# ajingu/RealSenseCalibration

Measured on NVIDIA B200. Metric: LM iterations/sec, higher is better.
Workload: dtype f64

## Files before the change

realsensecalibration_b200/csrc/ba_cuda.cu:

```cuda
#include <dlfcn.h>

#include <algorithm>
#include <atomic>
#include <chrono>
#include <cmath>
#include <string>

#include "ba_dense.cuh"
#include "ba_dense_blocked.cuh"
#include "ba_kernels.cuh"
#include "ba_structure.cuh"
#include "ba_rcs.cuh"
#include "ba_fused_a.cuh"
#include "ba_strip_a.cuh"
#include "ba_exchange.cuh"
#include "ba_rig.cuh"
#include "ba_cov.cuh"

using namespace ba;

namespace {
typedef struct ncclComm* ncclComm_t;
struct NcclUniqueId { char internal[128]; };
struct Nccl {
// ... 495 lines not shown
  }
  BA_LAUNCH(p, KT_CANDIDATE, (k_candidate<6>), gcf, 256, 0, S.nf, p->f_act_ptr.p, p->xf.p, p->sf.p, p->yf.p, p->xf_c.p, p->bp0.p, p->bp1.p);
  {
    FoldJob J = {{p->bp0.p, p->bp1.p, nullptr, nullptr}, {S_XF2, S_DF2, 0, 0}, {0, 0, 0, 0}};
    BA_LAUNCH(p, KT_FOLD, k_fold_multi, 2, 1024, 0, J, gcf, p->scal.p);
  }
  BA_CUDA_TRY(cudaGetLastError());
  fam_end(p, F_UPDATE);
  fam_begin(p, F_COST);
  BA_TRY(run_cost_candidate(p));
  fam_end(p, F_COST);
  return allreduce_step_scalars(p);
}

FaParams fa_params(ba_cuda_problem* p, const ba_cuda_options& opt) {
  const Structure& S = p->S;
  FusedA& F = p->FA;
  const size_t nt = (size_t)F.n_tiles;
  FaParams P;
  P.tiles = F.tiles.p; P.e_ptr = S.e_ptr.p; P.ob_f = S.ob_f0.p; P.uv = p->uv.p;
  P.ob_meta = p->use_strip ? p->SA.ob_meta.p : F.ob_meta.p;
  P.tile_cams = p->use_strip ? p->SA.strip_cams.p : F.cams.group_target.p; P.cap = F.cap;
  P.pts_cap = F.pts_cap; P.tcam = F.tcam; P.tcs = F.tcs; P.pent_cap = F.pent_cap;
  P.pitem_begin = F.pairs.item_begin.p; P.pitem_end = F.pairs.item_end.p; P.pent = F.pairs.ent.p;
  P.citem_begin = F.cams.item_begin.p; P.citem_end = F.cams.item_end.p; P.cent = F.cams.ent.p;
  P.xe = p->xe.p; P.se = p->se.p; P.tab_f = p->tab_f.p; P.radius = p->scal.p + S_RADIUS;
  P.min_diag = opt.min_lm_diagonal; P.max_diag = opt.max_lm_diagonal;
  P.partP = F.partP.p; P.partC = F.partC.p; P.Lz = F.Lz.p; P.se_out = p->se.p;
  P.cost_partial = p->fa_part.p; P.g2_partial = p->fa_part.p + nt; P.gmax_partial = p->fa_part.p + 2 * nt;
  P.yf = p->yf.p; P.tabc_f = p->tabc_f.p; P.xe_c = p->xe_c.p;
  P.mcc_partial = p->fa_part.p + 3 * nt; P.x2_partial = p->fa_part.p + 4 * nt; P.d2_partial = p->fa_part.p + 5 * nt;
  P.cand_partial = p->fa_part.p + 6 * nt;
  P.RES = p->RES.p; P.JE = p->JE.p; P.JF = p->JF0.p;
  P.status = p->status.p;
  P.loss = p->loss;
  return P;
}

int fa_set_smem_attr(ba_cuda_problem* p) {
  if (!p->smem_attr_set) {
    const int kMax = (int)FA_SMEM_MAX;
    BA_CUDA_TRY(cudaFuncSetAttribute(k_fa_pass1<FA_FULL>, cudaFuncAttributeMaxDynamicSharedMemorySize, kMax));
    BA_CUDA_TRY(cudaFuncSetAttribute(k_fa_pass1<FA_NORMS>, cudaFuncAttributeMaxDynamicSharedMemorySize, kMax));
    BA_CUDA_TRY(cudaFuncSetAttribute(k_fa_pass1<FA_GRAD>, cudaFuncAttributeMaxDynamicSharedMemorySize, kMax));
    BA_CUDA_TRY(cudaFuncSetAttribute(k_fa_pass1<FA_FIRST>, cudaFuncAttributeMaxDynamicSharedMemorySize, kMax));
    BA_CUDA_TRY(cudaFuncSetAttribute(k_fa_pass2, cudaFuncAttributeMaxDynamicSharedMemorySize, kMax));
    BA_CUDA_TRY(cudaFuncSetAttribute(k_fa_jac, cudaFuncAttributeMaxDynamicSharedMemorySize, kMax));
    BA_CUDA_TRY(cudaFuncSetAttribute(k_sa_pass1<SA_FULL>, cudaFuncAttributeMaxDynamicSharedMemorySize, kMax));
    BA_CUDA_TRY(cudaFuncSetAttribute(k_sa_pass1<SA_GRAD>, cudaFuncAttributeMaxDynamicSharedMemorySize, kMax));
    BA_CUDA_TRY(cudaFuncSetAttribute(k_sa_pass1<SA_FIRST>, cudaFuncAttributeMaxDynamicSharedMemorySize, kMax));
    p->smem_attr_set = true;
  }
  return BA_OK;
}

// ... 201 lines not shown
      LaunchScope scope(p, KT_RCS);
      BA_TRY(launch_pcg(p->pcg, p->R, p->Sb.p, p->rhs.p, p->yf.p, p->status.p, opt, p->st));
    }
    BA_CUDA_TRY(cudaMemcpyAsync(&p->h_pcg_iters, p->pcg.iters.p, sizeof(int), cudaMemcpyDeviceToHost, p->st));
  } else {
    if (p->use_strip)
      BA_LAUNCH(p, KT_ASSEMBLE, k_sa_diag_rhs_dense, grid_for(S.nf * 6, 128), 128, 0, S.nf, F.camacc.p, radius, opt.min_lm_diagonal,
                opt.max_lm_diagonal, n, p->Sd.p, p->rhs.p);
    else
      BA_LAUNCH(p, KT_ASSEMBLE, k_diag_rhs_dense, grid_for(S.nf * 6, 128), 128, 0, S.nf, F.camacc.p, FA_NVC, F.camacc.p + 27, FA_NVC, radius,
                opt.min_lm_diagonal, opt.max_lm_diagonal, n, p->Sd.p, p->rhs.p);
    LaunchScope scope(p, KT_RCS);
    BA_TRY(dense_solve(p, n));
  }
  fam_end(p, F_SOLVE);
  fam_begin(p, F_UPDATE);
  const int gcf = (int)grid_for(S.nf * 6, 256);
  BA_LAUNCH(p, KT_CANDIDATE, (k_candidate<6>), gcf, 256, 0, S.nf, p->f_act_ptr.p, p->xf.p, p->sf.p, p->yf.p, p->xf_c.p, p->bp0.p, p->bp1.p);
  {
    FoldJob J = {{p->bp0.p, p->bp1.p, nullptr, nullptr}, {S_XF2, S_DF2, 0, 0}, {0, 0, 0, 0}};
    BA_LAUNCH(p, KT_FOLD, k_fold_multi, 2, 1024, 0, J, gcf, p->scal.p);
  }
  BA_TRY(build_tables(p, true));
  const FaParams P = fa_params(p, opt);
  BA_LAUNCH(p, KT_FA_P2, k_fa_pass2, F.n_tiles, F.threads2, F.smem2(), P);
  {
    FoldJob J = {{P.mcc_partial, P.x2_partial, P.d2_partial, P.cand_partial}, {S_MCC, S_XE2, S_DE2, S_CAND}, {0, 0, 0, 0}};
    BA_LAUNCH(p, KT_FOLD, k_fold_multi, 4, 1024, 0, J, F.n_tiles, p->scal.p);
  }
  BA_CUDA_TRY(cudaGetLastError());
  fam_end(p, F_UPDATE);
  return allreduce_step_scalars(p);
}

bool lm_fused(const ba_cuda_problem* p) { return p->model == 0 && p->use_fused && !p->lm.opt.force_generic_path; }

int sx_prepare(ba_cuda_problem* p) {
  const Structure& S = p->S;
  SparseExchange& X = p->SX;
  X.on = false; X.world = p->world; X.nvc = p->use_strip ? SA_NVC : FA_NVC;
  if (!nccl().AllGather || !env_int("BA_SX", 0, 1, 1)) return BA_OK;
  cudaStream_t st = p->st;
  const int64_t nf = S.nf, nd = p->R.nd;
  DVec<int32_t> cflag, cpos, dflag, dpos;
  BA_TRY(cflag.alloc(nf + 1)); BA_TRY(cpos.alloc(nf + 1)); BA_TRY(dflag.alloc((size_t)S.ndest + 1)); BA_TRY(dpos.alloc((size_t)S.ndest + 1));
  BA_CUDA_TRY(cudaMemsetAsync(cflag.p, 0, sizeof(int32_t) * (nf + 1), st));
  BA_CUDA_TRY(cudaMemsetAsync(dflag.p, 0, sizeof(int32_t) * ((size_t)S.ndest + 1), st));
  k_sx_flags<<<grid_for(nf, 256), 256, 0, st>>>(S.fobs_ptr.p, nf, cflag.p);
// ... 1424 lines not shown
```

realsensecalibration_b200/csrc/ba_fused_a.cuh:

```cuda
#pragma once
#include <cuda_pipeline.h>

#include <chrono>
#include <cstdio>

#include "ba_kernels.cuh"
#include "ba_structure.cuh"

namespace ba {

constexpr int FA_TOBS_DEFAULT = 256;
constexpr int FA_KMAX = 64;
constexpr int FA_TPTS = 4096;
constexpr int FA_TCAM = 48;
constexpr int FA_CH_PAIR = 16;
constexpr int FA_CH_RED = 64;
constexpr int FA_NVC = 33;
constexpr int FA_MAX_THREADS = 512;
constexpr int FA_THREADS_DEFAULT = 128;
constexpr int FA_REC = 22;
constexpr int FA_REC2 = 10;
constexpr int FA_PENT_MAX = 6144;
constexpr size_t FA_SMEM_MAX = 231000;
constexpr int FA_LS = 10;
// ... 42 lines not shown
  DVec<int64_t> tile_item_ptr;
  DVec<int32_t> item_target;
  DVec<int32_t> red_items;
  DVec<int64_t> tgt_ptr;
  Chunks red_ch;
  DVec<int64_t> group_ptr;
  DVec<int32_t> group_target;
  DVec<int64_t> tile_group_ptr;
};

struct FusedA {
  bool ready = false;
  int n_tiles = 0, tobs = FA_TOBS_DEFAULT, kmax = 0, cap = 0, threads = FA_THREADS_DEFAULT, threads2 = FA_THREADS_DEFAULT, ch_cam = 16, ch_pair = FA_CH_PAIR;
  DVec<int64_t> tile_pt_ptr;
  DVec<int64_t> tile_pent_ptr;
  DVec<int64_t> tile_cent_ptr;
  ItemSet pairs, cams;
  DVec<uint32_t> ob_meta;
  DVec<FaTile> tiles;
  DVec<double> partP, partC, red1P, red1C, camacc, Lz;
  int pts_cap = FA_TPTS;
  int tcam = FA_TCAM;
  int tcs = FA_TCAM + 1;
  int pent_cap = 0;
  size_t smem1() const {
    return ((size_t)cap * FA_REC + (size_t)pts_cap * FA_LS + (size_t)tcs * TAB) * 8 + ((size_t)pent_cap + cap) * 4 + (size_t)cap * 2;
  }
  size_t smem2() const { return ((size_t)cap * FA_REC2 + (size_t)pts_cap * FA_PS2 + (size_t)tcs * (TAB + 16)) * 8; }
  size_t smemj(int threads) const { return ((size_t)threads * FA_RECJ + (size_t)pts_cap * FA_PS2 + (size_t)tcs * TAB) * 8 + (size_t)cap * 20; }
};

__global__ void k_fa_tile_flags(const int64_t* __restrict__ e_ptr, int64_t ne, int tobs, int32_t* __restrict__ flag, int* __restrict__ kmax) {
  const int64_t pt = blockIdx.x * (int64_t)blockDim.x + threadIdx.x;
  if (pt >= ne) return;
  atomicMax(kmax, (int)min(e_ptr[pt + 1] - e_ptr[pt], (int64_t)INT32_MAX));
  int f = 0;
  if (pt > 0) f = (e_ptr[pt] / tobs != e_ptr[pt - 1] / tobs) || (pt / FA_TPTS != (pt - 1) / FA_TPTS);
  flag[pt] = f;
}

__global__ void k_fa_pair_fill(const int64_t* __restrict__ e_ptr, const int32_t* __restrict__ ob_f, int64_t ne, int64_t nf,
                               const int64_t* __restrict__ off, const int32_t* __restrict__ tile_of_pt, const int64_t* __restrict__ tile_pt_ptr,
                               const uint64_t* __restrict__ dest_keys, int ndest, const uint64_t* __restrict__ dh_keys,
                               const int32_t* __restrict__ dh_val, uint64_t dh_mask, int dh_shift, uint64_t* __restrict__ keys,
                               int32_t* __restrict__ vals) {
  const int64_t e = blockIdx.x * (int64_t)blockDim.x + threadIdx.x;
  if (e >= ne) return;
  int64_t o = off[e];
  const int tile = tile_of_pt[e];
  const int64_t ob0 = e_ptr[tile_pt_ptr[tile]];
  for (int64_t i = e_ptr[e]; i < e_ptr[e + 1]; ++i)
// ... 256 lines not shown
inline int build_fused_a_tobs(FusedA& F, const Structure& S, cudaStream_t st, int tobs);

inline int build_fused_a(FusedA& F, const Structure& S, cudaStream_t st) {
  F.ready = false;
  if (S.ne == 0 || S.nb == 0 || S.nslots != 1) return BA_ERR_UNSUPPORTED;
  const int64_t np = S.npairs - S.nf;
  if (np >= (int64_t)INT32_MAX) return BA_ERR_UNSUPPORTED;
  const bool dense_pairs = (double)np >= 4.0 * (double)S.nb;
  int tobs = env_int("BA_FA_TOBS", 64, 1024, dense_pairs ? 1024 : 480);
  for (;; tobs /= 2) {
    F.threads = env_int("BA_FA_THREADS", 32, FA_MAX_THREADS, tobs >= 768 ? 512 : 256) / 32 * 32;
    F.threads2 = env_int("BA_FA_THREADS2", 32, FA_MAX_THREADS, tobs >= 768 ? 256 : 128) / 32 * 32;
    F.ch_cam = env_int("BA_FA_CH_CAM", 1, 63, 16);
    F.ch_pair = env_int("BA_FA_CH_PAIR", 1, 63, dense_pairs ? FA_CH_PAIR : 12);
    const int rc = build_fused_a_tobs(F, S, st, tobs);
    if (rc != BA_ERR_UNSUPPORTED || tobs <= 128 || F.kmax > FA_KMAX) return rc;
  }
}

inline int build_fused_a_tobs(FusedA& F, const Structure& S, cudaStream_t st, int tobs) {
  F.ready = false;
  const int64_t ne = S.ne, nb = S.nb, nf = S.nf;
  F.tobs = tobs;
  FaLap L(st);
  DVec<int32_t> flag, tile_of_pt;
  DVec<int> kmax;
  BA_TRY(flag.alloc(ne)); BA_TRY(tile_of_pt.alloc(ne)); BA_TRY(kmax.alloc_zero(1, st));
  k_fa_tile_flags<<<grid_for(ne, 256), 256, 0, st>>>(S.e_ptr.p, ne, F.tobs, flag.p, kmax.p);
  BA_TRY(cub_call([&](void* t, size_t& b) { return cub::DeviceScan::InclusiveSum(t, b, flag.p, tile_of_pt.p, (int)ne, st); }));
  int last_tile = 0;
  BA_CUDA_TRY(cudaMemcpyAsync(&F.kmax, kmax.p, sizeof(int), cudaMemcpyDeviceToHost, st));
  BA_CUDA_TRY(cudaMemcpyAsync(&last_tile, tile_of_pt.p + (ne - 1), sizeof(int32_t), cudaMemcpyDeviceToHost, st));
  BA_CUDA_TRY(cudaStreamSynchronize(st));
  if (F.kmax > FA_KMAX) return BA_ERR_UNSUPPORTED;
  F.cap = F.tobs + F.kmax;
  F.n_tiles = last_tile + 1;
  BA_TRY(F.tile_pt_ptr.alloc((size_t)F.n_tiles + 1));
  k_seg_ptr<int32_t><<<grid_for(ne > F.n_tiles + 1 ? ne : F.n_tiles + 1, 256), 256, 0, st>>>(tile_of_pt.p, ne, F.n_tiles, F.tile_pt_ptr.p);
  L.lap("tiles");
  int max_tile_cams = 0;
  {
    DVec<uint64_t> keys;
    DVec<int32_t> vals, group_tile;
    DVec<int> mx;
    BA_TRY(keys.alloc(nb)); BA_TRY(vals.alloc(nb)); BA_TRY(mx.alloc_zero(1, st));
    k_fa_cam_fill<<<grid_for(nb, 256), 256, 0, st>>>(S.ob_e.p, S.ob_f0.p, nb, nf, S.e_ptr.p, tile_of_pt.p, F.tile_pt_ptr.p, keys.p, vals.p);
// ... 62 lines not shown
    F.tcs = F.tcam | 1;
    F.pent_cap = std::min(h[2], FA_PENT_MAX);
    F.pent_cap += F.pent_cap & 1;
    if (F.smem1() > FA_SMEM_MAX) {
      const size_t excess = (F.smem1() - FA_SMEM_MAX + 7) / 8 * 2;
      F.pent_cap = (size_t)F.pent_cap > excess ? F.pent_cap - (int)excess : 0;
    }
    if (F.smem1() > FA_SMEM_MAX || F.smem2() > FA_SMEM_MAX || F.smemj(FA_JAC_THREADS) > FA_SMEM_MAX) return BA_ERR_UNSUPPORTED;
  }
  L.lap("pair items, geometry");
  BA_TRY(F.tiles.alloc((size_t)F.n_tiles));
  k_fa_tile_desc<<<grid_for(F.n_tiles, 256), 256, 0, st>>>(F.n_tiles, F.tile_pt_ptr.p, S.e_ptr.p, F.cams.tile_group_ptr.p, F.tile_pent_ptr.p,
                                                          F.tile_cent_ptr.p, F.pairs.tile_item_ptr.p, F.cams.tile_item_ptr.p, F.tiles.p);
  BA_TRY(F.partP.alloc((size_t)F.pairs.n_items * 36)); BA_TRY(F.partC.alloc((size_t)F.cams.n_items * FA_NVC));
  BA_TRY(F.red1P.alloc((size_t)F.pairs.red_ch.n * 36)); BA_TRY(F.red1C.alloc((size_t)F.cams.red_ch.n * FA_NVC));
  BA_TRY(F.camacc.alloc((size_t)nf * FA_NVC + 2 + 64));
  BA_TRY(F.Lz.alloc((size_t)ne * 9));
  BA_CUDA_TRY(cudaStreamSynchronize(st));
  BA_CUDA_TRY(cudaGetLastError());
  F.ready = true;
  return BA_OK;
}

__device__ __forceinline__ void fa_linearize(const double* __restrict__ T, const double* X, const double* s, double2 ob, double* r,
                                             double* je, double* jf) {
  double q[3];
  mat3_vec(T, X, q);
  const double p0 = q[0] + T[18], p1 = q[1] + T[19], p2 = q[2] + T[20];
  r[0] = T[21] * p0 / p2 + T[23] - ob.x;
  r[1] = T[22] * p1 / p2 + T[24] - ob.y;
  const double iz = 1.0 / p2;
  const double a = T[21] * iz, bb = -T[21] * p0 * iz * iz, cc = T[22] * iz, dd = -T[22] * p1 * iz * iz;
  double D[9];
  rot_deriv(T + 9, T[25] != 0.0 ? X : q, D);
#pragma unroll
  for (int k = 0; k < 3; ++k) {
    jf[k] = (a * D[k] + bb * D[6 + k]) * T[26 + k];
    jf[6 + k] = (cc * D[3 + k] + dd * D[6 + k]) * T[26 + k];
  }
  jf[3] = a * T[29]; jf[4] = 0.0;        jf[5] = bb * T[31];
  jf[9] = 0.0;       jf[10] = cc * T[30]; jf[11] = dd * T[31];
  je[0] = (a * T[0] + bb * T[6]) * s[0]; je[1] = (a * T[1] + bb * T[7]) * s[1]; je[2] = (a * T[2] + bb * T[8]) * s[2];
  je[3] = (cc * T[3] + dd * T[6]) * s[0]; je[4] = (cc * T[4] + dd * T[7]) * s[1]; je[5] = (cc * T[5] + dd * T[8]) * s[2];
}

__device__ __forceinline__ bool fa_chol3(const double* M , double* Lp) {
  const double d0 = M[0];
  if (!(d0 > 0.0) || !isfinite(d0)) return false;
  const double i0 = rsqrt(d0);
  const double l10 = M[1] * i0, l20 = M[2] * i0;
  const double d1 = M[3] - l10 * l10;
  if (!(d1 > 0.0) || !isfinite(d1)) return false;
  const double i1 = rsqrt(d1);
  const double l21 = (M[4] - l20 * l10) * i1;
  const double d2 = M[5] - l20 * l20 - l21 * l21;
  if (!(d2 > 0.0) || !isfinite(d2)) return false;
  Lp[0] = l10; Lp[1] = l20; Lp[2] = l21; Lp[3] = i0; Lp[4] = i1; Lp[5] = rsqrt(d2);
  return true;
}
__device__ __forceinline__ void fa_fwd3(const double* Lp, double* x) {
  x[0] *= Lp[3];
  x[1] = (x[1] - Lp[0] * x[0]) * Lp[4];
  x[2] = (x[2] - Lp[1] * x[0] - Lp[2] * x[1]) * Lp[5];
}
__device__ __forceinline__ void fa_bwd3(const double* Lp, double* x) {
  x[2] *= Lp[5];
  x[1] = (x[1] - Lp[2] * x[2]) * Lp[4];
  x[0] = (x[0] - Lp[0] * x[1] - Lp[1] * x[2]) * Lp[3];
}

struct FaParams {
  const FaTile* tiles;
  const int64_t* e_ptr; const int32_t* ob_f; const uint32_t* ob_meta; const double2* uv;
  const int32_t* tile_cams;
  const int64_t* pitem_begin; const int64_t* pitem_end; const int32_t* pent;
  const int64_t* citem_begin; const int64_t* citem_end; const int32_t* cent;
  int cap, pts_cap, tcam, tcs, pent_cap;
  const double* xe; const double* se; const double* tab_f; const double* radius;
  double min_diag, max_diag;
  double* partP; double* partC; double* Lz; double* se_out;
  double* cost_partial; double* gmax_partial; double* g2_partial;
  const double* yf; const double* tabc_f; double* xe_c;
  double* mcc_partial; double* x2_partial; double* d2_partial; double* cand_partial;
  double* RES; double* JE; double* JF;
  int* status;
  LossSpec loss;
};

__device__ __forceinline__ double fa_apply_loss(const LossSpec L, double* r, double* je, double* jf) {
  const double s = r[0] * r[0] + r[1] * r[1];
  if (L.type == 0) return s;
  double rho, w;
  loss_apply(L, s, &rho, &w);
  r[0] *= w; r[1] *= w;
#pragma unroll
  for (int k = 0; k < 6; ++k) je[k] *= w;
#pragma unroll
  for (int k = 0; k < 12; ++k) jf[k] *= w;
  return rho;
}

__device__ __forceinline__ FaTile fa_load_tile(const FaTile* __restrict__ p) {
  FaTile T;
  const int4* s = reinterpret_cast<const int4*>(p);
  int4* d = reinterpret_cast<int4*>(&T);
#pragma unroll
// ... 266 lines not shown
      const double2 rv = R2[9], wv = R2[10];
      int c = 0;
#pragma unroll
      for (int a = 0; a < 6; ++a)
#pragma unroll
        for (int b = a; b < 6; ++b) acc[c++] += jf[a] * jf[b] + jf[6 + a] * jf[6 + b];
#pragma unroll
      for (int a = 0; a < 6; ++a) { acc[21 + a] += jf[a] * rv.x + jf[6 + a] * rv.y; acc[27 + a] += jf[a] * wv.x + jf[6 + a] * wv.y; }
    }
    double* out = P.partC + (size_t)it * FA_NVC;
#pragma unroll
    for (int k = 0; k < FA_NVC; ++k) out[k] = acc[k];
  }
  if (!NORMS) {
    double v[3] = {sq, g2, gmx};
    const bool mx[3] = {false, false, true};
    fa_block_reduce(v, mx, 3, red);
    if (tid == 0) { P.cost_partial[tile] = v[0]; P.g2_partial[tile] = v[1]; P.gmax_partial[tile] = v[2]; }
  }
}

__device__ __constant__ int kFaCandFields[16] = {0, 1, 2, 3, 4, 5, 6, 7, 8, 18, 19, 20, 21, 22, 23, 24};

__global__ void __launch_bounds__(FA_MAX_THREADS, 1) k_fa_pass2(FaParams P) {
  extern __shared__ double smem[];
  double* rec = smem;
  double* Xs = rec + (size_t)P.cap * FA_REC2;
  double* tabs = Xs + (size_t)P.pts_cap * FA_PS2;
  double* tabc = tabs + (size_t)P.tcs * TAB;
  __shared__ double red[128];
  const int tile = blockIdx.x, tid = threadIdx.x, nthr = blockDim.x;
  const FaTile T = fa_load_tile(P.tiles + tile);
  const int64_t pt0 = T.pt0, ob0 = T.ob0;
  const int nobs = T.nobs, npts = T.npts;
  fa_stage_tables_async(P, T, P.tab_f, tabs, TAB, nullptr);
  for (int i = tid; i < 3 * npts; i += nthr) {
    const int lp = i / 3, k = i - 3 * lp;
    __pipeline_memcpy_async(Xs + lp * FA_PS2 + k, P.xe + 3 * pt0 + i, 8);
    __pipeline_memcpy_async(Xs + lp * FA_PS2 + 3 + k, P.se + 3 * pt0 + i, 8);
  }
  __pipeline_commit();
  fa_stage_tables_async(P, T, P.tabc_f, tabc, 16, kFaCandFields);
  __pipeline_commit();
  int pl0 = 0, pl1 = 0;
  if (tid < npts) {
    pl0 = (int)(P.e_ptr[pt0 + tid] - ob0);
    pl1 = (int)(P.e_ptr[pt0 + tid + 1] - ob0);
  }
  uint32_t m_n = 0;
  int32_t c_n = 0;
  double2 uv_n = make_double2(0.0, 0.0);
  if (tid < nobs) { m_n = P.ob_meta[ob0 + tid]; c_n = P.ob_f[ob0 + tid]; uv_n = P.uv[ob0 + tid]; }
  __pipeline_wait_prior(1);
  __syncthreads();
  for (int l = tid; l < nobs; l += nthr) {
    const int lp = (int)(m_n & 0xffffu), slot = (int)(m_n >> 16);
    const int32_t c = c_n;
    const double2 ob = uv_n;
    if (l + nthr < nobs) { const int64_t o = ob0 + l + nthr; m_n = P.ob_meta[o]; c_n = P.ob_f[o]; uv_n = P.uv[o]; }
    double y[6];
#pragma unroll
    for (int k = 0; k < 6; ++k) y[k] = __ldg(P.yf + 6 * (int64_t)c + k);
    double Tt[TAB];
    fa_get_table(P, tabs, P.tab_f, slot, c, Tt);
    const double* xs = Xs + lp * FA_PS2;
    const double X[3] = {xs[0], xs[1], xs[2]};
    const double s[3] = {xs[3], xs[4], xs[5]};
    double r[2], je[6], jf[12];
    fa_linearize(Tt, X, s, ob, r, je, jf);
    fa_apply_loss(P.loss, r, je, jf);
    double q0 = 0.0, q1 = 0.0;
#pragma unroll
    for (int k = 0; k < 6; ++k) { q0 += jf[k] * y[k]; q1 += jf[6 + k] * y[k]; }
    double2* R2 = reinterpret_cast<double2*>(rec + (size_t)l * FA_REC2);
#pragma unroll
    for (int k = 0; k < 3; ++k) R2[k] = make_double2(je[2 * k], je[2 * k + 1]);
    R2[3] = make_double2(r[0], r[1]);
    R2[4] = make_double2(q0, q1);
  }
  uint32_t m2 = 0;
  double2 uv2 = make_double2(0.0, 0.0);
  if (tid < nobs) { m2 = P.ob_meta[ob0 + tid]; uv2 = P.uv[ob0 + tid]; }
  __syncthreads();
  double mcc = 0.0, x2 = 0.0, d2 = 0.0;
  for (int lp = tid; lp < npts; lp += nthr) {
    const int64_t e = pt0 + lp;
    int l0 = pl0, l1 = pl1;
    if (lp != tid) { l0 = (int)(P.e_ptr[e] - ob0); l1 = (int)(P.e_ptr[e + 1] - ob0); }
    const double* in = P.Lz + 9 * e;
    double Lp[6], t[3];
#pragma unroll
    for (int k = 0; k < 6; ++k) Lp[k] = in[k];
#pragma unroll
    for (int k = 0; k < 3; ++k) t[k] = in[6 + k];
    for (int l = l0; l < l1; ++l) {
      const double* R = rec + (size_t)l * FA_REC2;
#pragma unroll
      for (int rr = 0; rr < 2; ++rr) {
        double u[3] = {R[3 * rr], R[3 * rr + 1], R[3 * rr + 2]};
        fa_fwd3(Lp, u);
        const double q = R[8 + rr];
        t[0] -= u[0] * q; t[1] -= u[1] * q; t[2] -= u[2] * q;
      }
    }
    fa_bwd3(Lp, t);
    for (int l = l0; l < l1; ++l) {
      const double* R = rec + (size_t)l * FA_REC2;
#pragma unroll
      for (int rr = 0; rr < 2; ++rr) {
        const double m = -(R[3 * rr] * t[0] + R[3 * rr + 1] * t[1] + R[3 * rr + 2] * t[2]) - R[8 + rr];
        mcc += m * (R[6 + rr] + m / 2.0);
      }
    }
    double* xs = Xs + lp * FA_PS2;
#pragma unroll
    for (int k = 0; k < 3; ++k) {
      const double xv = xs[k];
      const double c = xv + (-(t[k]) * xs[3 + k]);
      P.xe_c[3 * e + k] = c;
      xs[k] = c;
      if (l1 > l0) { x2 += xv * xv; const double d = xv - c; d2 += d * d; }
    }
  }
  __pipeline_wait_prior(0);
  __syncthreads();
  double sq = 0.0;
  for (int l = tid; l < nobs; l += nthr) {
    const int lp = (int)(m2 & 0xffffu), slot = (int)(m2 >> 16);
    const double2 ob = uv2;
    if (l + nthr < nobs) { const int64_t o = ob0 + l + nthr; m2 = P.ob_meta[o]; uv2 = P.uv[o]; }
    double C[16];
    if (slot < P.tcam) {
#pragma unroll
      for (int f = 0; f < 16; ++f) C[f] = fa_table_field(tabc, P.tcs, f, slot);
    } else {
      const double* Tc = P.tabc_f + TAB * (int64_t)P.ob_f[ob0 + l];
#pragma unroll
      for (int f = 0; f < 16; ++f) C[f] = __ldg(Tc + kFaCandFields[f]);
    }
    const double* xs = Xs + lp * FA_PS2;
    const double X[3] = {xs[0], xs[1], xs[2]};
    double q[3];
    mat3_vec(C, X, q);
    const double p0 = q[0] + C[9], p1 = q[1] + C[10], p2 = q[2] + C[11];
    const double r0 = C[12] * p0 / p2 + C[14] - ob.x;
    const double r1 = C[13] * p1 / p2 + C[15] - ob.y;
    double sc = r0 * r0 + r1 * r1;
    if (P.loss.type != 0) { double w; loss_apply(P.loss, sc, &sc, &w); }
    sq += sc;
  }
  double v[4] = {mcc, x2, d2, sq};
  const bool mx[4] = {false, false, false, false};
  fa_block_reduce(v, mx, 4, red);
  if (tid == 0) { P.mcc_partial[tile] = v[0]; P.x2_partial[tile] = v[1]; P.d2_partial[tile] = v[2]; P.cand_partial[tile] = v[3]; }
}

__global__ void __launch_bounds__(FA_JAC_THREADS, 4) k_fa_jac(FaParams P) {
  extern __shared__ double smem[];
  const int tile = blockIdx.x, tid = threadIdx.x, nthr = blockDim.x, lane = tid & 31, warp = tid >> 5;
  double* wje = smem + (size_t)warp * (32 * FA_RECJ);
  double* wjf = wje + 32 * 6;
  double2* uv_s = reinterpret_cast<double2*>(smem + (size_t)(nthr >> 5) * (32 * FA_RECJ));
  double* Xs = reinterpret_cast<double*>(uv_s + P.cap);
  double* tabs = Xs + (size_t)P.pts_cap * FA_PS2;
  uint32_t* meta_s = reinterpret_cast<uint32_t*>(tabs + (size_t)P.tcs * TAB);
  __shared__ double red[32];
  const FaTile T = fa_load_tile(P.tiles + tile);
  const int64_t pt0 = T.pt0, ob0 = T.ob0;
  const int nobs = T.nobs, npts = T.npts;
  fa_stage_tables_async(P, T, P.tab_f, tabs, TAB, nullptr);
  for (int i = tid; i < 3 * npts; i += nthr) {
    const int lp = i / 3, k = i - 3 * lp;
    __pipeline_memcpy_async(Xs + lp * FA_PS2 + k, P.xe + 3 * pt0 + i, 8);
    __pipeline_memcpy_async(Xs + lp * FA_PS2 + 3 + k, P.se + 3 * pt0 + i, 8);
  }
  for (int i = tid; i < nobs; i += nthr) {
    __pipeline_memcpy_async(uv_s + i, P.uv + ob0 + i, 16);
// ... 140 lines not shown
```

realsensecalibration_b200/csrc/ba_strip_a.cuh:

```cuda
#pragma once
#include "ba_fused_a.cuh"

namespace ba {

constexpr int SA_NT = 512;
constexpr int SA_NCS_MAX = 64;
constexpr int SA_NVC = 39;
constexpr int SA_REC = 22;
constexpr int SA_NF_CAP = 1024;
constexpr int SA_POS_MAX = 4096;
constexpr int SA_CM_MAX = 8;
constexpr int SA_TYPE_IDLE = 0, SA_TYPE_PAIR = 1, SA_TYPE_FLUSH = 2, SA_TYPE_CAM = 3;
constexpr int SA_FULL = 0, SA_GRAD = 2, SA_FIRST = 3;

__host__ __device__ inline int sa_xs_len(int pts_cap) { return (3 * pts_cap + 4 + 1) & ~1; }

struct __align__(16) SaTile {
  int64_t pt0, ob0, pos0, ent0, pidx0, fout0;
  int32_t npts, nobs, npos, nent;
};
static_assert(sizeof(SaTile) == 64, "SaTile is loaded as four 16-byte words");
struct __align__(16) SaStrip {
  int64_t cam0, pout0, cout0;
  int32_t tile0, ntiles, ncs, nflush;
// ... 770 lines not shown
  const int64_t n_pblocks = A.n_pout + A.n_fout;
  if (n_pblocks >= (int64_t)INT32_MAX / 64 || A.n_cout >= (int64_t)INT32_MAX / 64) return BA_ERR_UNSUPPORTED;
  {
    DVec<int32_t> ptarget, ctarget, iota;
    BA_TRY(ptarget.alloc((size_t)n_pblocks)); BA_TRY(ctarget.alloc((size_t)A.n_cout));
    k_sa_targets_persist<<<grid_for((int64_t)ns * SA_NT, 256), 256, 0, st>>>(ns, A.strips.p, A.slot_out.p, slot_dest.p, A.strip_cams.p, nf,
                                                                            S.dh_keys.p, S.dh_val.p, S.dh_mask, S.dh_shift, ptarget.p, ctarget.p);
    k_sa_targets_flush<<<grid_for(nt, 4), 128, 0, st>>>(nt, L, A.segw, nf_cap, A.tiles.p, A.strips.p, A.seg.p, fl_dest.p, A.strip_cams.p, nf,
                                                       S.dh_keys.p, S.dh_val.p, S.dh_mask, S.dh_shift, A.n_pout, ptarget.p);
    const int64_t nmax = std::max(n_pblocks, A.n_cout);
    BA_TRY(iota.alloc((size_t)nmax));
    k_iota<<<grid_for(nmax, 256), 256, 0, st>>>(iota.p, nmax, 0);
    BA_TRY(sort_to_csr(ptarget.p, iota.p, n_pblocks, S.ndest, A.tgt_ptr_p, A.red_items_p, st));
    BA_TRY(build_chunks(A.red_ch_p, A.tgt_ptr_p.p, S.ndest, FA_CH_RED, st));
    BA_TRY(sort_to_csr(ctarget.p, iota.p, A.n_cout, nf, A.tgt_ptr_c, A.red_items_c, st));
    BA_TRY(build_chunks(A.red_ch_c, A.tgt_ptr_c.p, (int)nf, FA_CH_RED, st));
    BA_CUDA_TRY(cudaStreamSynchronize(st));
  }
  Lp.lap("strip: reduction lists");
  BA_TRY(A.partP.alloc((size_t)n_pblocks * 36)); BA_TRY(A.partC.alloc((size_t)A.n_cout * SA_NVC));
  BA_TRY(A.red1P.alloc((size_t)A.red_ch_p.n * 36)); BA_TRY(A.red1C.alloc((size_t)A.red_ch_c.n * SA_NVC));
  F.n_tiles = nt; F.tobs = tobs; F.kmax = A.kmax; F.cap = std::max(A.nobs_cap, 1);
  F.threads = SA_NT; F.threads2 = env_int("BA_FA_THREADS2", 32, FA_MAX_THREADS, tobs >= 640 ? 256 : 128) / 32 * 32;
  F.pts_cap = A.pts_cap; F.tcam = std::min(A.ncs_cap, FA_TCAM); F.tcs = F.tcam | 1; F.pent_cap = 0;
  if (F.smem2() > FA_SMEM_MAX || F.smemj(FA_JAC_THREADS) > FA_SMEM_MAX) return BA_ERR_UNSUPPORTED;
  BA_TRY(F.tiles.alloc((size_t)nt));
  k_sa_fa_tiles<<<grid_for(nt, 256), 256, 0, st>>>(nt, L, A.tiles.p, A.strips.p, F.tiles.p);
  BA_TRY(F.camacc.alloc((size_t)nf * SA_NVC + 2 + 64));
  BA_TRY(F.Lz.alloc((size_t)ne * 9));
  BA_CUDA_TRY(cudaStreamSynchronize(st));
  BA_CUDA_TRY(cudaGetLastError());
  if (Lp.on)
    std::fprintf(stderr, "[ba_cuda timing]   strip geometry: tobs %d L %d tiles %d strips %d | positions %d points %d cameras %d entries staged %d of %d "
                         "owner slots %d | smem %zu B | blocks: %lld per strip + %lld flushed, %lld camera\n", tobs, L, nt, ns, A.cap_pos, A.pts_cap,
                 A.ncs_cap, A.ent_cap, max_nent, A.segw, A.smem(), (long long)A.n_pout, (long long)A.n_fout, (long long)A.n_cout);
  A.ready = true; F.ready = true;
  return BA_OK;
}

struct SaParams {
  const SaStrip* strips; const SaTile* tiles; const int32_t* strip_cams; const uint32_t* slot_out;
  const uint32_t* pm; const double2* puv; const uint16_t* pidx; const int32_t* ent; const uint16_t* seg;
  int segw, cap_pos, pts_cap, tcs, ent_cap, pidx_cap;
  const double* xe; const double* se; const double* tab_f; const double* radius;
  double min_diag, max_diag;
  double* partP; double* partC; int64_t n_pout;
  double* Lz; double* se_out; double* cost_partial; double* g2_partial; double* gmax_partial; int* status;
// ... 413 lines not shown
```

Measured before the change: 118.4.

## Process a whole strip of tiles per block in fused pass 2, reusing staged camera tables

Pass 2 now launches one block per strip of L tiles, not one per tile. Camera tables, candidate tables and camera step vectors are staged into shared memory once per strip and reused across its tiles, and the next tile descriptor is prefetched asynchronously. Point offsets and observation metadata are staged into shared memory, the mcc accumulation is split into a separate pass, and linearisation reads table fields directly rather than copying them into registers first. Optional clock64 instrumentation is added behind an environment flag. The cost is fewer, longer-running blocks (less parallelism), a larger shared-memory footprint because the camera cap is no longer clamped, and an extra barrier and pass per tile.

```diff
diff --git a/realsensecalibration_b200/csrc/ba_cuda.cu b/realsensecalibration_b200/csrc/ba_cuda.cu
--- a/realsensecalibration_b200/csrc/ba_cuda.cu
+++ b/realsensecalibration_b200/csrc/ba_cuda.cu
@@ -541,6 +541,7 @@
   P.ob_meta = p->use_strip ? p->SA.ob_meta.p : F.ob_meta.p;
   P.tile_cams = p->use_strip ? p->SA.strip_cams.p : F.cams.group_target.p; P.cap = F.cap;
   P.pts_cap = F.pts_cap; P.tcam = F.tcam; P.tcs = F.tcs; P.pent_cap = F.pent_cap;
+  P.n_tiles = F.n_tiles; P.tiles2 = F.tiles2;
   P.pitem_begin = F.pairs.item_begin.p; P.pitem_end = F.pairs.item_end.p; P.pent = F.pairs.ent.p;
   P.citem_begin = F.cams.item_begin.p; P.citem_end = F.cams.item_end.p; P.cent = F.cams.ent.p;
   P.xe = p->xe.p; P.se = p->se.p; P.tab_f = p->tab_f.p; P.radius = p->scal.p + S_RADIUS;
@@ -550,6 +551,7 @@
   P.yf = p->yf.p; P.tabc_f = p->tabc_f.p; P.xe_c = p->xe_c.p;
   P.mcc_partial = p->fa_part.p + 3 * nt; P.x2_partial = p->fa_part.p + 4 * nt; P.d2_partial = p->fa_part.p + 5 * nt;
   P.cand_partial = p->fa_part.p + 6 * nt;
+  P.clocks2 = nullptr;
   P.RES = p->RES.p; P.JE = p->JE.p; P.JF = p->JF0.p;
   P.status = p->status.p;
   P.loss = p->loss;
@@ -797,8 +799,23 @@
     BA_LAUNCH(p, KT_FOLD, k_fold_multi, 2, 1024, 0, J, gcf, p->scal.p);
   }
   BA_TRY(build_tables(p, true));
-  const FaParams P = fa_params(p, opt);
-  BA_LAUNCH(p, KT_FA_P2, k_fa_pass2, F.n_tiles, F.threads2, F.smem2(), P);
+  FaParams P = fa_params(p, opt);
+  static DVec<unsigned long long>* clk = nullptr;
+  if (env_int("BA_FA2_CLOCKS", 0, 1, 0)) {
+    if (!clk) { clk = new DVec<unsigned long long>(); BA_TRY(clk->alloc(5)); }
+    BA_CUDA_TRY(cudaMemsetAsync(clk->p, 0, 5 * sizeof(unsigned long long), p->st));
+    P.clocks2 = clk->p;
+  }
+  BA_LAUNCH(p, KT_FA_P2, k_fa_pass2, (F.n_tiles + F.tiles2 - 1) / F.tiles2, F.threads2, F.smem2(), P);
+  if (P.clocks2) {
+    unsigned long long h[5];
+    BA_CUDA_TRY(cudaMemcpyAsync(h, P.clocks2, sizeof(h), cudaMemcpyDeviceToHost, p->st));
+    BA_CUDA_TRY(cudaStreamSynchronize(p->st));
+    const double n = (double)F.n_tiles;
+    std::fprintf(stderr, "[ba_cuda clocks] pass 2, cycles per tile as thread 0 sees them: prologue + staging %.0f | observations + barrier %.0f | "
+                         "points + barrier %.0f | candidate %.0f | reduction %.0f | sum %.0f\n", h[0] / n, h[1] / n, h[2] / n, h[3] / n, h[4] / n,
+                 (h[0] + h[1] + h[2] + h[3] + h[4]) / n);
+  }
   {
     FoldJob J = {{P.mcc_partial, P.x2_partial, P.d2_partial, P.cand_partial}, {S_MCC, S_XE2, S_DE2, S_CAND}, {0, 0, 0, 0}};
     BA_LAUNCH(p, KT_FOLD, k_fold_multi, 4, 1024, 0, J, F.n_tiles, p->scal.p);
diff --git a/realsensecalibration_b200/csrc/ba_fused_a.cuh b/realsensecalibration_b200/csrc/ba_fused_a.cuh
--- a/realsensecalibration_b200/csrc/ba_fused_a.cuh
+++ b/realsensecalibration_b200/csrc/ba_fused_a.cuh
@@ -88,11 +88,15 @@
   int pts_cap = FA_TPTS;
   int tcam = FA_TCAM;
   int tcs = FA_TCAM + 1;
+  int tiles2 = 1;
   int pent_cap = 0;
   size_t smem1() const {
     return ((size_t)cap * FA_REC + (size_t)pts_cap * FA_LS + (size_t)tcs * TAB) * 8 + ((size_t)pent_cap + cap) * 4 + (size_t)cap * 2;
   }
-  size_t smem2() const { return ((size_t)cap * FA_REC2 + (size_t)pts_cap * FA_PS2 + (size_t)tcs * (TAB + 16)) * 8; }
+  size_t smem2() const {
+    return ((size_t)cap * FA_REC2 + (size_t)tcam * 6 + (size_t)tcs * (TAB + 16) + (size_t)pts_cap * (FA_PS2 + 1) + 1) * 8 +
+           (size_t)cap * 4;
+  }
   size_t smemj(int threads) const { return ((size_t)threads * FA_RECJ + (size_t)pts_cap * FA_PS2 + (size_t)tcs * TAB) * 8 + (size_t)cap * 20; }
 };
 
@@ -395,6 +399,7 @@
   F.ready = false;
   const int64_t ne = S.ne, nb = S.nb, nf = S.nf;
   F.tobs = tobs;
+  F.tiles2 = 1;
   FaLap L(st);
   DVec<int32_t> flag, tile_of_pt;
   DVec<int> kmax;
@@ -503,17 +508,25 @@
   return BA_OK;
 }
 
-__device__ __forceinline__ void fa_linearize(const double* __restrict__ T, const double* X, const double* s, double2 ob, double* r,
-                                             double* je, double* jf) {
-  double q[3];
-  mat3_vec(T, X, q);
+template <typename Tab>
+__device__ __forceinline__ void fa_linearize(const Tab& T, const double* X, const double* s, double2 ob, double* r, double* je, double* jf) {
+  const double q[3] = {T[0] * X[0] + T[1] * X[1] + T[2] * X[2], T[3] * X[0] + T[4] * X[1] + T[5] * X[2],
+                       T[6] * X[0] + T[7] * X[1] + T[8] * X[2]};
   const double p0 = q[0] + T[18], p1 = q[1] + T[19], p2 = q[2] + T[20];
   r[0] = T[21] * p0 / p2 + T[23] - ob.x;
   r[1] = T[22] * p1 / p2 + T[24] - ob.y;
   const double iz = 1.0 / p2;
   const double a = T[21] * iz, bb = -T[21] * p0 * iz * iz, cc = T[22] * iz, dd = -T[22] * p1 * iz * iz;
+  const bool small = T[25] != 0.0;
+  const double b[3] = {small ? X[0] : q[0], small ? X[1] : q[1], small ? X[2] : q[2]};
   double D[9];
-  rot_deriv(T + 9, T[25] != 0.0 ? X : q, D);
+#pragma unroll
+  for (int k = 0; k < 3; ++k) {
+    const double a0 = T[9 + k], a1 = T[12 + k], a2 = T[15 + k];
+    D[k] = a1 * b[2] - a2 * b[1];
+    D[3 + k] = a2 * b[0] - a0 * b[2];
+    D[6 + k] = a0 * b[1] - a1 * b[0];
+  }
 #pragma unroll
   for (int k = 0; k < 3; ++k) {
     jf[k] = (a * D[k] + bb * D[6 + k]) * T[26 + k];
@@ -557,12 +570,14 @@
   const int64_t* pitem_begin; const int64_t* pitem_end; const int32_t* pent;
   const int64_t* citem_begin; const int64_t* citem_end; const int32_t* cent;
   int cap, pts_cap, tcam, tcs, pent_cap;
+  int n_tiles, tiles2;
   const double* xe; const double* se; const double* tab_f; const double* radius;
   double min_diag, max_diag;
   double* partP; double* partC; double* Lz; double* se_out;
   double* cost_partial; double* gmax_partial; double* g2_partial;
   const double* yf; const double* tabc_f; double* xe_c;
   double* mcc_partial; double* x2_partial; double* d2_partial; double* cand_partial;
+  unsigned long long* clocks2;
   double* RES; double* JE; double* JF;
   int* status;
   LossSpec loss;
@@ -875,137 +890,191 @@
 
 __device__ __constant__ int kFaCandFields[16] = {0, 1, 2, 3, 4, 5, 6, 7, 8, 18, 19, 20, 21, 22, 23, 24};
 
+struct FaPlaneTab {
+  const double* tabs; int tcs, slot;
+  __device__ __forceinline__ double operator[](int f) const { return fa_table_field(tabs, tcs, f, slot); }
+};
+struct FaGlobalTab {
+  const double* t;
+  __device__ __forceinline__ double operator[](int f) const { return __ldg(t + f); }
+};
+struct FaGlobalCandTab {
+  const double* t;
+  __device__ __forceinline__ double operator[](int f) const { return __ldg(t + kFaCandFields[f]); }
+};
+
+template <typename Tab>
+__device__ __forceinline__ double fa_cand_cost(const Tab& C, const double* X, double2 ob, const LossSpec L) {
+  const double q[3] = {C[0] * X[0] + C[1] * X[1] + C[2] * X[2], C[3] * X[0] + C[4] * X[1] + C[5] * X[2],
+                       C[6] * X[0] + C[7] * X[1] + C[8] * X[2]};
+  const double p0 = q[0] + C[9], p1 = q[1] + C[10], p2 = q[2] + C[11];
+  const double r0 = C[12] * p0 / p2 + C[14] - ob.x;
+  const double r1 = C[13] * p1 / p2 + C[15] - ob.y;
+  double sc = r0 * r0 + r1 * r1;
+  if (L.type != 0) { double w; loss_apply(L, sc, &sc, &w); }
+  return sc;
+}
+
 __global__ void __launch_bounds__(FA_MAX_THREADS, 1) k_fa_pass2(FaParams P) {
-  extern __shared__ double smem[];
+  extern __shared__ __align__(128) double smem[];
   double* rec = smem;
-  double* Xs = rec + (size_t)P.cap * FA_REC2;
-  double* tabs = Xs + (size_t)P.pts_cap * FA_PS2;
+  double* ys = rec + (size_t)P.cap * FA_REC2;
+  double* tabs = ys + (size_t)P.tcam * 6;
   double* tabc = tabs + (size_t)P.tcs * TAB;
+  double* Xs = tabc + (size_t)P.tcs * 16;
+  int64_t* eps = reinterpret_cast<int64_t*>(Xs + (size_t)P.pts_cap * FA_PS2);
+  uint32_t* meta_s = reinterpret_cast<uint32_t*>(eps + P.pts_cap + 1);
   __shared__ double red[128];
-  const int tile = blockIdx.x, tid = threadIdx.x, nthr = blockDim.x;
-  const FaTile T = fa_load_tile(P.tiles + tile);
-  const int64_t pt0 = T.pt0, ob0 = T.ob0;
-  const int nobs = T.nobs, npts = T.npts;
-  fa_stage_tables_async(P, T, P.tab_f, tabs, TAB, nullptr);
-  for (int i = tid; i < 3 * npts; i += nthr) {
-    const int lp = i / 3, k = i - 3 * lp;
-    __pipeline_memcpy_async(Xs + lp * FA_PS2 + k, P.xe + 3 * pt0 + i, 8);
-    __pipeline_memcpy_async(Xs + lp * FA_PS2 + 3 + k, P.se + 3 * pt0 + i, 8);
-  }
-  __pipeline_commit();
-  fa_stage_tables_async(P, T, P.tabc_f, tabc, 16, kFaCandFields);
-  __pipeline_commit();
-  int pl0 = 0, pl1 = 0;
-  if (tid < npts) {
-    pl0 = (int)(P.e_ptr[pt0 + tid] - ob0);
-    pl1 = (int)(P.e_ptr[pt0 + tid + 1] - ob0);
-  }
-  uint32_t m_n = 0;
-  int32_t c_n = 0;
-  double2 uv_n = make_double2(0.0, 0.0);
-  if (tid < nobs) { m_n = P.ob_meta[ob0 + tid]; c_n = P.ob_f[ob0 + tid]; uv_n = P.uv[ob0 + tid]; }
-  __pipeline_wait_prior(1);
-  __syncthreads();
-  for (int l = tid; l < nobs; l += nthr) {
-    const int lp = (int)(m_n & 0xffffu), slot = (int)(m_n >> 16);
-    const int32_t c = c_n;
-    const double2 ob = uv_n;
-    if (l + nthr < nobs) { const int64_t o = ob0 + l + nthr; m_n = P.ob_meta[o]; c_n = P.ob_f[o]; uv_n = P.uv[o]; }
-    double y[6];
-#pragma unroll
-    for (int k = 0; k < 6; ++k) y[k] = __ldg(P.yf + 6 * (int64_t)c + k);
-    double Tt[TAB];
-    fa_get_table(P, tabs, P.tab_f, slot, c, Tt);
-    const double* xs = Xs + lp * FA_PS2;
-    const double X[3] = {xs[0], xs[1], xs[2]};
-    const double s[3] = {xs[3], xs[4], xs[5]};
-    double r[2], je[6], jf[12];
-    fa_linearize(Tt, X, s, ob, r, je, jf);
-    fa_apply_loss(P.loss, r, je, jf);
-    double q0 = 0.0, q1 = 0.0;
-#pragma unroll
-    for (int k = 0; k < 6; ++k) { q0 += jf[k] * y[k]; q1 += jf[6 + k] * y[k]; }
-    double2* R2 = reinterpret_cast<double2*>(rec + (size_t)l * FA_REC2);
-#pragma unroll
-    for (int k = 0; k < 3; ++k) R2[k] = make_double2(je[2 * k], je[2 * k + 1]);
-    R2[3] = make_double2(r[0], r[1]);
-    R2[4] = make_double2(q0, q1);
-  }
-  uint32_t m2 = 0;
-  double2 uv2 = make_double2(0.0, 0.0);
-  if (tid < nobs) { m2 = P.ob_meta[ob0 + tid]; uv2 = P.uv[ob0 + tid]; }
-  __syncthreads();
-  double mcc = 0.0, x2 = 0.0, d2 = 0.0;
-  for (int lp = tid; lp < npts; lp += nthr) {
-    const int64_t e = pt0 + lp;
-    int l0 = pl0, l1 = pl1;
-    if (lp != tid) { l0 = (int)(P.e_ptr[e] - ob0); l1 = (int)(P.e_ptr[e + 1] - ob0); }
-    const double* in = P.Lz + 9 * e;
-    double Lp[6], t[3];
-#pragma unroll
-    for (int k = 0; k < 6; ++k) Lp[k] = in[k];
-#pragma unroll
-    for (int k = 0; k < 3; ++k) t[k] = in[6 + k];
-    for (int l = l0; l < l1; ++l) {
-      const double* R = rec + (size_t)l * FA_REC2;
-#pragma unroll
-      for (int rr = 0; rr < 2; ++rr) {
-        double u[3] = {R[3 * rr], R[3 * rr + 1], R[3 * rr + 2]};
-        fa_fwd3(Lp, u);
-        const double q = R[8 + rr];
-        t[0] -= u[0] * q; t[1] -= u[1] * q; t[2] -= u[2] * q;
-      }
-    }
-    fa_bwd3(Lp, t);
-    for (int l = l0; l < l1; ++l) {
-      const double* R = rec + (size_t)l * FA_REC2;
+  __shared__ FaTile Tnext[2];
+  const int tid = threadIdx.x, nthr = blockDim.x;
+  __shared__ long long ck[6];
+  auto tick = [&](int k) { if (P.clocks2 && tid == 0) ck[k] = clock64(); };
+  const int tile0 = blockIdx.x * P.tiles2, tile1 = min(tile0 + P.tiles2, P.n_tiles);
+  FaTile T = fa_load_tile(P.tiles + tile0);
+  for (int tile = tile0; tile < tile1; ++tile) {
+    if (tile != tile0) T = Tnext[tile & 1];
+    tick(0);
+    const int64_t pt0 = T.pt0, ob0 = T.ob0;
+    const int nobs = T.nobs, npts = T.npts;
+    if (tile == tile0) {
+      fa_stage_tables_async(P, T, P.tab_f, tabs, TAB, nullptr);
+      for (int s = tid; s < min(T.ncam, P.tcam); s += nthr) {
+        const int64_t cam = __ldg(P.tile_cams + T.cam0 + s);
+#pragma unroll
+        for (int k = 0; k < 3; ++k) __pipeline_memcpy_async(ys + 6 * s + 2 * k, P.yf + 6 * cam + 2 * k, 16);
+      }
+    }
+    if (tid < 6 && tile + 1 < tile1)
+      __pipeline_memcpy_async(reinterpret_cast<int4*>(&Tnext[(tile + 1) & 1]) + tid, reinterpret_cast<const int4*>(P.tiles + tile + 1) + tid, 16);
+    for (int i = tid; i < 3 * npts; i += nthr) {
+      const int lp = i / 3, k = i - 3 * lp;
+      __pipeline_memcpy_async(Xs + lp * FA_PS2 + k, P.xe + 3 * pt0 + i, 8);
+      __pipeline_memcpy_async(Xs + lp * FA_PS2 + 3 + k, P.se + 3 * pt0 + i, 8);
+    }
+    for (int i = tid; i <= npts; i += nthr) __pipeline_memcpy_async(eps + i, P.e_ptr + pt0 + i, 8);
+    for (int i = tid; i < nobs; i += nthr) __pipeline_memcpy_async(meta_s + i, P.ob_meta + ob0 + i, 4);
+    __pipeline_commit();
+    if (tile == tile0) fa_stage_tables_async(P, T, P.tabc_f, tabc, 16, kFaCandFields);
+    __pipeline_commit();
+    double2 uv_n = make_double2(0.0, 0.0);
+    if (tid < nobs) uv_n = P.uv[ob0 + tid];
+    __pipeline_wait_prior(1);
+    __syncthreads();
+    tick(1);
+    for (int l = tid; l < nobs; l += nthr) {
+      const uint32_t m = meta_s[l];
+      const int lp = (int)(m & 0xffffu), slot = (int)(m >> 16);
+      const double2 ob = uv_n;
+      if (l + nthr < nobs) uv_n = P.uv[ob0 + l + nthr];
+      const double* xs = Xs + lp * FA_PS2;
+      const double X[3] = {xs[0], xs[1], xs[2]};
+      const double s[3] = {xs[3], xs[4], xs[5]};
+      double r[2], je[6], jf[12], y[6];
+      if (slot < P.tcam) {
+        const double2* y2 = reinterpret_cast<const double2*>(ys + 6 * slot);
+#pragma unroll
+        for (int k = 0; k < 3; ++k) { const double2 v = y2[k]; y[2 * k] = v.x; y[2 * k + 1] = v.y; }
+        fa_linearize(FaPlaneTab{tabs, P.tcs, slot}, X, s, ob, r, je, jf);
+      } else {
+        const int64_t c = P.ob_f[ob0 + l];
+#pragma unroll
+        for (int k = 0; k < 6; ++k) y[k] = __ldg(P.yf + 6 * c + k);
+        fa_linearize(FaGlobalTab{P.tab_f + TAB * c}, X, s, ob, r, je, jf);
+      }
+      fa_apply_loss(P.loss, r, je, jf);
+      double q0 = 0.0, q1 = 0.0;
+#pragma unroll
+      for (int k = 0; k < 6; ++k) { q0 += jf[k] * y[k]; q1 += jf[6 + k] * y[k]; }
+      double2* R2 = reinterpret_cast<double2*>(rec + (size_t)l * FA_REC2);
+#pragma unroll
+      for (int k = 0; k < 3; ++k) R2[k] = make_double2(je[2 * k], je[2 * k + 1]);
+      R2[3] = make_double2(r[0], r[1]);
+      R2[4] = make_double2(q0, q1);
+    }
+    double2 uv2 = make_double2(0.0, 0.0);
+    if (tid < nobs) uv2 = P.uv[ob0 + tid];
+    double Lz0[9];
+    if (tid < npts) {
+#pragma unroll
+      for (int k = 0; k < 9; ++k) Lz0[k] = P.Lz[9 * (pt0 + tid) + k];
+    }
+    __syncthreads();
+    tick(2);
+    double x2 = 0.0, d2 = 0.0;
+    for (int lp = tid; lp < npts; lp += nthr) {
+      const int64_t e = pt0 + lp;
+      const int l0 = (int)(eps[lp] - ob0), l1 = (int)(eps[lp + 1] - ob0);
+      if (lp != tid) {
+#pragma unroll
+        for (int k = 0; k < 9; ++k) Lz0[k] = P.Lz[9 * e + k];
+      }
+      const double Lp[6] = {Lz0[0], Lz0[1], Lz0[2], Lz0[3], Lz0[4], Lz0[5]};
+      double t[3] = {Lz0[6], Lz0[7], Lz0[8]};
+      for (int l = l0; l < l1; ++l) {
+        const double* R = rec + (size_t)l * FA_REC2;
+#pragma unroll
+        for (int rr = 0; rr < 2; ++rr) {
+          double u[3] = {R[3 * rr], R[3 * rr + 1], R[3 * rr + 2]};
+          fa_fwd3(Lp, u);
+          const double q = R[8 + rr];
+          t[0] -= u[0] * q; t[1] -= u[1] * q; t[2] -= u[2] * q;
+        }
+      }
+      fa_bwd3(Lp, t);
+      double* xs = Xs + lp * FA_PS2;
+#pragma unroll
+      for (int k = 0; k < 3; ++k) {
+        const double xv = xs[k];
+        const double c = xv + (-(t[k]) * xs[3 + k]);
+        P.xe_c[3 * e + k] = c;
+        xs[k] = c;
+        xs[3 + k] = t[k];
+        if (l1 > l0) { x2 += xv * xv; const double d = xv - c; d2 += d * d; }
+      }
+    }
+    __pipeline_wait_prior(0);
+    __syncthreads();
+    tick(3);
+    double sq = 0.0;
+    for (int l = tid; l < nobs; l += nthr) {
+      const uint32_t mt = meta_s[l];
+      const int lp = (int)(mt & 0xffffu), slot = (int)(mt >> 16);
+      const double2 ob = uv2;
+      if (l + nthr < nobs) uv2 = P.uv[ob0 + l + nthr];
+      const double* xs = Xs + lp * FA_PS2;
+      const double* t = xs + 3;
+      double* R = rec + (size_t)l * FA_REC2;
 #pragma unroll
       for (int rr = 0; rr < 2; ++rr) {
         const double m = -(R[3 * rr] * t[0] + R[3 * rr + 1] * t[1] + R[3 * rr + 2] * t[2]) - R[8 + rr];
-        mcc += m * (R[6 + rr] + m / 2.0);
-      }
-    }
-    double* xs = Xs + lp * FA_PS2;
-#pragma unroll
-    for (int k = 0; k < 3; ++k) {
-      const double xv = xs[k];
-      const double c = xv + (-(t[k]) * xs[3 + k]);
-      P.xe_c[3 * e + k] = c;
-      xs[k] = c;
-      if (l1 > l0) { x2 += xv * xv; const double d = xv - c; d2 += d * d; }
-    }
-  }
-  __pipeline_wait_prior(0);
-  __syncthreads();
-  double sq = 0.0;
-  for (int l = tid; l < nobs; l += nthr) {
-    const int lp = (int)(m2 & 0xffffu), slot = (int)(m2 >> 16);
-    const double2 ob = uv2;
-    if (l + nthr < nobs) { const int64_t o = ob0 + l + nthr; m2 = P.ob_meta[o]; uv2 = P.uv[o]; }
-    double C[16];
-    if (slot < P.tcam) {
-#pragma unroll
-      for (int f = 0; f < 16; ++f) C[f] = fa_table_field(tabc, P.tcs, f, slot);
-    } else {
-      const double* Tc = P.tabc_f + TAB * (int64_t)P.ob_f[ob0 + l];
-#pragma unroll
-      for (int f = 0; f < 16; ++f) C[f] = __ldg(Tc + kFaCandFields[f]);
-    }
-    const double* xs = Xs + lp * FA_PS2;
-    const double X[3] = {xs[0], xs[1], xs[2]};
-    double q[3];
-    mat3_vec(C, X, q);
-    const double p0 = q[0] + C[9], p1 = q[1] + C[10], p2 = q[2] + C[11];
-    const double r0 = C[12] * p0 / p2 + C[14] - ob.x;
-    const double r1 = C[13] * p1 / p2 + C[15] - ob.y;
-    double sc = r0 * r0 + r1 * r1;
-    if (P.loss.type != 0) { double w; loss_apply(P.loss, sc, &sc, &w); }
-    sq += sc;
-  }
-  double v[4] = {mcc, x2, d2, sq};
-  const bool mx[4] = {false, false, false, false};
-  fa_block_reduce(v, mx, 4, red);
-  if (tid == 0) { P.mcc_partial[tile] = v[0]; P.x2_partial[tile] = v[1]; P.d2_partial[tile] = v[2]; P.cand_partial[tile] = v[3]; }
+        R[8 + rr] = m;
+      }
+      const double X[3] = {xs[0], xs[1], xs[2]};
+      if (slot < P.tcam) sq += fa_cand_cost(FaPlaneTab{tabc, P.tcs, slot}, X, ob, P.loss);
+      else sq += fa_cand_cost(FaGlobalCandTab{P.tabc_f + TAB * (int64_t)P.ob_f[ob0 + l]}, X, ob, P.loss);
+    }
+    __syncthreads();
+    tick(4);
+    double mcc = 0.0;
+    for (int lp = tid; lp < npts; lp += nthr) {
+      const int l0 = (int)(eps[lp] - ob0), l1 = (int)(eps[lp + 1] - ob0);
+      for (int l = l0; l < l1; ++l) {
+        const double* R = rec + (size_t)l * FA_REC2;
+#pragma unroll
+        for (int rr = 0; rr < 2; ++rr) {
+          const double m = R[8 + rr];
+          mcc += m * (R[6 + rr] + m / 2.0);
+        }
+      }
+    }
+    double v[4] = {mcc, x2, d2, sq};
+    const bool mx[4] = {false, false, false, false};
+    fa_block_reduce(v, mx, 4, red);
+    if (tid == 0) { P.mcc_partial[tile] = v[0]; P.x2_partial[tile] = v[1]; P.d2_partial[tile] = v[2]; P.cand_partial[tile] = v[3]; }
+    tick(5);
+    if (P.clocks2 && tid == 0)
+      for (int k = 0; k < 5; ++k) atomicAdd(P.clocks2 + k, (unsigned long long)(ck[k + 1] - ck[k]));
+  }
 }
 
 __global__ void __launch_bounds__(FA_JAC_THREADS, 4) k_fa_jac(FaParams P) {
diff --git a/realsensecalibration_b200/csrc/ba_strip_a.cuh b/realsensecalibration_b200/csrc/ba_strip_a.cuh
--- a/realsensecalibration_b200/csrc/ba_strip_a.cuh
+++ b/realsensecalibration_b200/csrc/ba_strip_a.cuh
@@ -816,7 +816,7 @@
   BA_TRY(A.red1P.alloc((size_t)A.red_ch_p.n * 36)); BA_TRY(A.red1C.alloc((size_t)A.red_ch_c.n * SA_NVC));
   F.n_tiles = nt; F.tobs = tobs; F.kmax = A.kmax; F.cap = std::max(A.nobs_cap, 1);
   F.threads = SA_NT; F.threads2 = env_int("BA_FA_THREADS2", 32, FA_MAX_THREADS, tobs >= 640 ? 256 : 128) / 32 * 32;
-  F.pts_cap = A.pts_cap; F.tcam = std::min(A.ncs_cap, FA_TCAM); F.tcs = F.tcam | 1; F.pent_cap = 0;
+  F.pts_cap = A.pts_cap; F.tcam = A.ncs_cap; F.tcs = F.tcam | 1; F.pent_cap = 0; F.tiles2 = L;
   if (F.smem2() > FA_SMEM_MAX || F.smemj(FA_JAC_THREADS) > FA_SMEM_MAX) return BA_ERR_UNSUPPORTED;
   BA_TRY(F.tiles.alloc((size_t)nt));
   k_sa_fa_tiles<<<grid_for(nt, 256), 256, 0, st>>>(nt, L, A.tiles.p, A.strips.p, F.tiles.p);
```

Result: faster. 122.6, median of 6 (+3.5%).
